# stijnherfst/Tyrant

Hardware: AMD Instinct MI355X
Metric: Mrays/s at 1080p 8spp (higher is better)
Workload: dtype f32

## Files before the change

tyrant_amd/csrc/hip/traverse.hpp:

```cpp
#pragma once

#include <type_traits>

#include <hip/hip_runtime.h>

#include "vecmath.hpp"

namespace tyr {

constexpr uint32_t kRefLeaf = 0x80000000u;
constexpr uint32_t kRefDone = 0xFFFFFFFFu;
constexpr uint32_t kRefPop = 0xFFFFFFFEu;
constexpr int kStackSize = 64;
constexpr uint32_t kMaxLeafPrims = 31;
constexpr uint32_t kMaxPrimOffset = 1u << 26;
constexpr uint32_t kStagedNodes = 64;
constexpr uint32_t kQuadOrderShift = 25;
constexpr uint32_t kQuadIndexMask = (1u << kQuadOrderShift) - 1u;

struct DevScene {
	const float4* quads;
	uint32_t quadRootRef;
	uint32_t nQuads;
	uint32_t nStaged;
	uint32_t quadMaxStack;
	const float4* nodes;
	const float4* tris;
	float rootMin[3];
	float rootMax[3];
	uint32_t rootRef;
	uint32_t nPairs;
	uint32_t nPrims;
};

#ifdef __HIPCC__

struct RayConst {
	f3 o, d, inv;
	bool nx, ny, nz;
};

__device__ __forceinline__ RayConst make_ray(f3 o, f3 d) {
	RayConst r;
	r.o = o;
	r.d = d;
	r.inv = mk3(1.f / d.x, 1.f / d.y, 1.f / d.z);
	r.nx = r.inv.x < 0;
	r.ny = r.inv.y < 0;
	r.nz = r.inv.z < 0;
	return r;
}

__device__ __forceinline__ bool slab_test(const RayConst& r, float lox, float hix, float loy, float hiy, float loz, float hiz, float lowest, float& tMinOut) {
	float tMin = (lox - r.o.x) * r.inv.x;
	float tMax = (hix - r.o.x) * r.inv.x;
	const float tyMin = (loy - r.o.y) * r.inv.y;
	const float tyMax = (hiy - r.o.y) * r.inv.y;
	bool ok = !(tMin > tyMax || tyMin > tMax);
	if (tyMin > tMin)
		tMin = tyMin;
	if (tyMax < tMax)
		tMax = tyMax;
	const float tzMin = (loz - r.o.z) * r.inv.z;
	const float tzMax = (hiz - r.o.z) * r.inv.z;
	ok = ok && !(tMin > tzMax || tzMin > tMax);
	if (tzMin > tMin)
		tMin = tzMin;
	if (tzMax < tMax)
		tMax = tzMax;
	tMinOut = tMin;
	return ok && (tMin < lowest) && (tMax > 0);
}

struct TriData {
	float4 a, b, c;
};
__device__ __forceinline__ TriData triangle_load(const float4* __restrict__ tris, uint32_t prim) {
	TriData d;
	d.a = tris[3 * prim + 0];
	d.b = tris[3 * prim + 1];
	d.c = tris[3 * prim + 2];
	return d;
}
__device__ __forceinline__ float triangle_test(const TriData& d, const RayConst& r);
__device__ __forceinline__ float triangle_test(const float4* __restrict__ tris, uint32_t prim, const RayConst& r) { return triangle_test(triangle_load(tris, prim), r); }
__device__ __forceinline__ float triangle_test(const TriData& d, const RayConst& r) {
	const float4 a = d.a, b = d.b, c = d.c;
	const f3 vert = mk3(a.x, a.y, a.z);
	const f3 e1 = mk3(a.w, b.x, b.y);
	const f3 e2 = mk3(b.z, b.w, c.x);
	const f3 pvec = cross(r.d, e2);
	const float det = dot(e1, pvec);
	if (det < 0.0000001f)
		return 0.0f;
	const float invDet = 1 / det;
	const f3 tvec = r.o - vert;
	const float u = dot(tvec, pvec) * invDet;
	if (u < 0 || u > 1)
		return 0.0f;
	const f3 qvec = cross(tvec, e1);
	const float v = dot(r.d, qvec) * invDet;
	if (v < 0 || u + v > 1)
		return 0.0f;
	return dot(e2, qvec) * invDet;
}
__device__ __forceinline__ float triangle_test_uv(const TriData& d, const RayConst& r, float& uOut, float& vOut) {
	const float4 a = d.a, b = d.b, c = d.c;
	const f3 vert = mk3(a.x, a.y, a.z);
	const f3 e1 = mk3(a.w, b.x, b.y);
	const f3 e2 = mk3(b.z, b.w, c.x);
	const f3 pvec = cross(r.d, e2);
	const float det = dot(e1, pvec);
	if (det < 0.0000001f)
		return 0.0f;
	const float invDet = 1 / det;
	const f3 tvec = r.o - vert;
	const float u = dot(tvec, pvec) * invDet;
	if (u < 0 || u > 1)
		return 0.0f;
	const f3 qvec = cross(tvec, e1);
	const float v = dot(r.d, qvec) * invDet;
	if (v < 0 || u + v > 1)
		return 0.0f;
	uOut = u;
	vOut = v;
	return dot(e2, qvec) * invDet;
}

__device__ __forceinline__ float triangle_test_select(const TriData& d, const RayConst& r) {
	const float4 a = d.a, b = d.b, c = d.c;
	const f3 vert = mk3(a.x, a.y, a.z);
	const f3 e1 = mk3(a.w, b.x, b.y);
	const f3 e2 = mk3(b.z, b.w, c.x);
	const f3 pvec = cross(r.d, e2);
	const float det = dot(e1, pvec);
	const bool out0 = det < 0.0000001f;
	const float invDet = 1 / det;
	const f3 tvec = r.o - vert;
	const float u = dot(tvec, pvec) * invDet;
	const bool out1 = u < 0 || u > 1;
	const f3 qvec = cross(tvec, e1);
	const float v = dot(r.d, qvec) * invDet;
	const bool out2 = v < 0 || u + v > 1;
	const float t = dot(e2, qvec) * invDet;
	return (out0 || out1 || out2) ? 0.0f : t;
}

template <int LDS_DEPTH>
struct TravStack {
	static constexpr int kBlockThreads = 256;
	static constexpr int kSpill = kStackSize - LDS_DEPTH;
	uint2* lds;
	uint32_t* spillRef;
	float* spillT;
	int n;
	uint32_t topRef;
	float topT;
	bool hasTop;
	bool overflow;
	__device__ __forceinline__ void bind(uint2* ldsColumn, uint32_t* refs, float* ts) {
		lds = ldsColumn;
		spillRef = refs;
		spillT = ts;
	}
	__device__ __forceinline__ void reset() {
		n = 0;
		hasTop = false;
		overflow = false;
	}
	__device__ __forceinline__ void push(uint32_t r, float t) {
		if (hasTop) {
			if (LDS_DEPTH > 0 && n < LDS_DEPTH) {
				lds[n * kBlockThreads] = make_uint2(topRef, __float_as_uint(topT));
				++n;
			} else if (n < kStackSize - 1) {
				spillRef[n - LDS_DEPTH] = topRef;
				spillT[n - LDS_DEPTH] = topT;
				++n;
			} else {
				overflow = true;
			}
		}
		topRef = r;
		topT = t;
		hasTop = true;
	}
	__device__ __forceinline__ bool pop(uint32_t& r, float& t) {
		if (hasTop) {
			r = topRef;
			t = topT;
			hasTop = false;
			return true;
		}
		if (n == 0)
			return false;
		--n;
		if (LDS_DEPTH > 0 && n < LDS_DEPTH) {
			const uint2 e = lds[n * kBlockThreads];
			r = e.x;
			t = __uint_as_float(e.y);
		} else {
			r = spillRef[n - LDS_DEPTH];
			t = spillT[n - LDS_DEPTH];
		}
		return true;
	}
};

template <int LDS_DEPTH, bool WITH_T = true>
struct LdsStack {
	static constexpr int kBlockThreads = 256;
	typedef typename std::conditional<WITH_T, uint2, uint32_t>::type entry_t;
#if defined(__HIP_DEVICE_COMPILE__)
	typedef __attribute__((address_space(3))) entry_t* lds_column_t;
#else
	typedef entry_t* lds_column_t;
#endif
	lds_column_t lds;
	uint32_t* spillRef;
	float* spillT;
	int n;
	bool overflow;
	__device__ __forceinline__ void bind(entry_t* ldsColumn, uint32_t* refs, float* ts) {
		lds = (lds_column_t)ldsColumn;
		spillRef = refs;
		spillT = ts;
	}
	__device__ __forceinline__ void reset() {
		n = 0;
		overflow = false;
	}
	__device__ __forceinline__ void lds_put(int d, uint32_t r, float t) {
		if constexpr (WITH_T)
			lds[d * kBlockThreads] = make_uint2(r, __float_as_uint(t));
		else
			lds[d * kBlockThreads] = r;
	}
	__device__ __forceinline__ void lds_get(int d, uint32_t& r, float& t) {
		if constexpr (WITH_T) {
			const uint2 e = lds[d * kBlockThreads];
			r = e.x;
			t = __uint_as_float(e.y);
		} else {
			r = lds[d * kBlockThreads];
			t = -__builtin_inff();
		}
	}
	__device__ __forceinline__ void push(uint32_t r, float t) {
		if (LDS_DEPTH > 0 && n < LDS_DEPTH) {
			lds_put(n, r, t);
			++n;
		} else if (n < kStackSize) {
			spillRef[n - LDS_DEPTH] = r;
			if (WITH_T)
				spillT[n - LDS_DEPTH] = t;
			++n;
		} else {
			overflow = true;
		}
	}
	__device__ __forceinline__ bool pop(uint32_t& r, float& t) {
		if (n == 0)
			return false;
		if (LDS_DEPTH > 0 && __builtin_amdgcn_ballot_w64(n > LDS_DEPTH) == 0ull) {
			--n;
			lds_get(n, r, t);
			return true;
		}
		--n;
		if (LDS_DEPTH > 0 && n < LDS_DEPTH) {
			lds_get(n, r, t);
		} else {
			r = spillRef[n - LDS_DEPTH];
			t = WITH_T ? spillT[n - LDS_DEPTH] : -__builtin_inff();
		}
		return true;
	}
	__device__ __forceinline__ void pop_select(bool popping, uint32_t& ref, float bound) {
		if (LDS_DEPTH > 0 && __builtin_amdgcn_ballot_w64(popping && n > LDS_DEPTH) == 0ull) {
			const bool take = popping && n > 0;
			uint32_t r;
			float t;
			lds_get(take ? n - 1 : 0, r, t);
			ref = popping ? (n == 0 ? kRefDone : (t < bound ? r : kRefPop)) : ref;
			n = take ? n - 1 : n;
			return;
		}
		if (popping) {
			if (n == 0) {
				ref = kRefDone;
			} else {
				--n;
				uint32_t r;
				float t;
				if (LDS_DEPTH > 0 && n < LDS_DEPTH) {
					lds_get(n, r, t);
				} else {
					r = spillRef[n - LDS_DEPTH];
					t = WITH_T ? spillT[n - LDS_DEPTH] : -__builtin_inff();
				}
				if (t < bound)
					ref = r;
			}
		}
	}
	__device__ __forceinline__ void push_ranked(const uint32_t* ref, const float* t, const unsigned long long* hit, const uint32_t* rank, uint32_t hr, uint32_t first) {
		if (LDS_DEPTH >= 3 && __builtin_amdgcn_ballot_w64(n > LDS_DEPTH - 3) == 0ull) {
			const uint32_t after = hr >> 1;
#pragma unroll
			for (int s = 0; s < 4; ++s)
				if (__builtin_amdgcn_inverse_ballot_w64(hit[s]) && rank[s] != first)
					lds_put(n + (int)__popc(after >> rank[s]), ref[s], t[s]);
			n += (int)__popc(hr) - (hr != 0u ? 1 : 0);
			return;
		}
		uint32_t oref[4];
		float ot[4];
#pragma unroll
		for (uint32_t k = 1; k < 4; ++k) {
			oref[k] = rank[0] == k ? ref[0] : rank[1] == k ? ref[1] : rank[2] == k ? ref[2] : ref[3];
			ot[k] = rank[0] == k ? t[0] : rank[1] == k ? t[1] : rank[2] == k ? t[2] : t[3];
		}
		if ((hr & 8u) && (hr & 7u))
			push(oref[3], ot[3]);
		if ((hr & 4u) && (hr & 3u))
			push(oref[2], ot[2]);
		if ((hr & 2u) && (hr & 1u))
			push(oref[1], ot[1]);
	}
	__device__ __forceinline__ void push3(unsigned long long ma, uint32_t ra, float ta, unsigned long long mb, uint32_t rb, float tb, unsigned long long mc, uint32_t rc, float tc) {
		if (LDS_DEPTH >= 3 && __builtin_amdgcn_ballot_w64(n > LDS_DEPTH - 3) == 0ull) {
			if (__builtin_amdgcn_inverse_ballot_w64(ma)) {
				lds_put(n, ra, ta);
				++n;
			}
			if (__builtin_amdgcn_inverse_ballot_w64(mb)) {
				lds_put(n, rb, tb);
				++n;
			}
			if (__builtin_amdgcn_inverse_ballot_w64(mc)) {
				lds_put(n, rc, tc);
				++n;
			}
			return;
		}
		if (__builtin_amdgcn_inverse_ballot_w64(ma))
			push(ra, ta);
		if (__builtin_amdgcn_inverse_ballot_w64(mb))
			push(rb, tb);
		if (__builtin_amdgcn_inverse_ballot_w64(mc))
			push(rc, tc);
	}
};

struct PairTest {
	uint32_t nearRef, farRef;
	float nearT, farT;
	bool nearHit, farHit;
	bool synthetic;
};

__device__ __forceinline__ PairTest test_pair(const float4* __restrict__ nodes, uint32_t idx, const RayConst& r, float dist) {
	const float4 qx = nodes[4 * idx + 0];
	const float4 qy = nodes[4 * idx + 1];
	const float4 qz = nodes[4 * idx + 2];
	const float4 qr = nodes[4 * idx + 3];
	const uint32_t leftRef = __float_as_uint(qr.x), rightRef = __float_as_uint(qr.y), axis = __float_as_uint(qr.z);
	float tL, tR;
	const bool hL = slab_test(r, r.nx ? qx.y : qx.x, r.nx ? qx.x : qx.y, r.ny ? qy.y : qy.x, r.ny ? qy.x : qy.y, r.nz ? qz.y : qz.x, r.nz ? qz.x : qz.y, dist, tL);
	const bool hR = slab_test(r, r.nx ? qx.w : qx.z, r.nx ? qx.z : qx.w, r.ny ? qy.w : qy.z, r.ny ? qy.z : qy.w, r.nz ? qz.w : qz.z, r.nz ? qz.z : qz.w, dist, tR);
	const bool rightFirst = (axis == 0) ? r.nx : (axis == 1) ? r.ny : (axis == 2) ? r.nz : false;
	PairTest p;
	p.nearRef = rightFirst ? rightRef : leftRef;
	p.farRef = rightFirst ? leftRef : rightRef;
	p.nearT = rightFirst ? tR : tL;
	p.farT = rightFirst ? tL : tR;
	p.nearHit = rightFirst ? hR : hL;
	p.farHit = rightFirst ? hL : hR;
	p.synthetic = (axis == 3);
	if (p.synthetic) {
		p.nearHit = true;
		p.farHit = true;
		p.farT = -__builtin_inff();
	}
	return p;
}


typedef float v2f __attribute__((ext_vector_type(2)));
__device__ __forceinline__ bool slab_fast(const RayConst& r, float lox, float hix, float loy, float hiy, float loz, float hiz, float lowest, float& tMinOut) {
	const float ox = r.o.x, oy = r.o.y, oz = r.o.z, ix = r.inv.x, iy = r.inv.y, iz = r.inv.z;
	v2f x = { lox, hix }, y = { loy, hiy }, z = { loz, hiz };
	x = (x - ox) * ix;
	y = (y - oy) * iy;
	z = (z - oz) * iz;
	const float tMin = __builtin_fmaxf(__builtin_fmaxf(__builtin_fminf(x.x, x.y), __builtin_fminf(y.x, y.y)), __builtin_fminf(z.x, z.y));
	const float tMax = __builtin_fminf(__builtin_fminf(__builtin_fmaxf(x.x, x.y), __builtin_fmaxf(y.x, y.y)), __builtin_fmaxf(z.x, z.y));
	tMinOut = tMin;
	return (tMin <= tMax) && (tMin < lowest) && (tMax > 0);
}
typedef unsigned long long lanemask;
__device__ __forceinline__ lanemask slab_fast_mask(const RayConst& r, float lox, float hix, float loy, float hiy, float loz, float hiz, float lowest, float& tMinOut) {
	const float ox = r.o.x, oy = r.o.y, oz = r.o.z, ix = r.inv.x, iy = r.inv.y, iz = r.inv.z;
	v2f x = { lox, hix }, y = { loy, hiy }, z = { loz, hiz };
	x = (x - ox) * ix;
	y = (y - oy) * iy;
	z = (z - oz) * iz;
	const float tMin = __builtin_fmaxf(__builtin_fmaxf(__builtin_fminf(x.x, x.y), __builtin_fminf(y.x, y.y)), __builtin_fminf(z.x, z.y));
	const float tMax = __builtin_fminf(__builtin_fminf(__builtin_fmaxf(x.x, x.y), __builtin_fmaxf(y.x, y.y)), __builtin_fmaxf(z.x, z.y));
	tMinOut = tMin;
	return __builtin_amdgcn_ballot_w64(tMin <= tMax) & __builtin_amdgcn_ballot_w64(tMin < lowest) & __builtin_amdgcn_ballot_w64(tMax > 0);
}
__device__ __forceinline__ bool ray_is_regular(const RayConst& r) {
	return (fabsf(r.inv.x) < __builtin_inff()) && (fabsf(r.inv.y) < __builtin_inff()) && (fabsf(r.inv.z) < __builtin_inff());
}
__device__ __forceinline__ PairTest test_pair_fast(const float4* __restrict__ nodes, uint32_t idx, const RayConst& r, float dist) {
	const float4 qx = nodes[4 * idx + 0];
	const float4 qy = nodes[4 * idx + 1];
	const float4 qz = nodes[4 * idx + 2];
	const float4 qr = nodes[4 * idx + 3];
	const uint32_t leftRef = __float_as_uint(qr.x), rightRef = __float_as_uint(qr.y), axis = __float_as_uint(qr.z);
	float tL, tR;
	const bool hL = slab_fast(r, qx.x, qx.y, qy.x, qy.y, qz.x, qz.y, dist, tL);
	const bool hR = slab_fast(r, qx.z, qx.w, qy.z, qy.w, qz.z, qz.w, dist, tR);
	const bool rightFirst = (axis == 0) ? r.nx : (axis == 1) ? r.ny : (axis == 2) ? r.nz : false;
	PairTest p;
	p.nearRef = rightFirst ? rightRef : leftRef;
	p.farRef = rightFirst ? leftRef : rightRef;
	p.nearT = rightFirst ? tR : tL;
	p.farT = rightFirst ? tL : tR;
	p.nearHit = rightFirst ? hR : hL;
	p.farHit = rightFirst ? hL : hR;
	p.synthetic = (axis == 3);
	if (p.synthetic) {
		p.nearHit = true;
		p.farHit = true;
		p.farT = -__builtin_inff();
	}
	return p;
}


__device__ __forceinline__ lanemask lanes_where(bool p) { return __builtin_amdgcn_ballot_w64(p); }
__device__ __forceinline__ bool lane_in(lanemask m) { return __builtin_amdgcn_inverse_ballot_w64(m); }
__device__ __forceinline__ lanemask mask_select(lanemask sel, lanemask a, lanemask b) { return (sel & a) | (~sel & b); }

__device__ __forceinline__ bool ref_is_leaf(uint32_t ref) { return (ref & kRefLeaf) && ref < kRefPop; }
__device__ __forceinline__ lanemask lanes_traversing(uint32_t ref) { return __builtin_amdgcn_ballot_w64((int)ref >= 0) | __builtin_amdgcn_ballot_w64(ref == kRefPop); }
__device__ __forceinline__ lanemask lanes_at_leaf(uint32_t ref) { return __builtin_amdgcn_ballot_w64((ref & kRefLeaf) != 0u) & __builtin_amdgcn_ballot_w64(ref < kRefPop); }

struct QuadHits {
	uint32_t ref[4];
	float t[4];
	lanemask hit[4];
};

template <bool FAST>
__device__ __forceinline__ lanemask slab_any(const RayConst& r, float lox, float hix, float loy, float hiy, float loz, float hiz, float lowest, float& tOut) {
	if (FAST)
		return slab_fast_mask(r, lox, hix, loy, hiy, loz, hiz, lowest, tOut);
	return lanes_where(slab_test(r, r.nx ? hix : lox, r.nx ? lox : hix, r.ny ? hiy : loy, r.ny ? loy : hiy, r.nz ? hiz : loz, r.nz ? loz : hiz, lowest, tOut));
}

template <bool FAST, bool ORDERED, bool STAGED = false, int STAGE_STRIDE = (int)kStagedNodes>
__device__ __forceinline__ QuadHits test_quad(const float4* __restrict__ quads, uint32_t ref, const RayConst& r, float dist, const float4* staged = nullptr, uint32_t nStaged = 0) {
	const uint32_t idx = ref & kQuadIndexMask;
	const float4* q = quads + 8 * idx;
	const uint32_t meta = ref >> kQuadOrderShift;
	float4 x01, x23, y01, y23, z01, z23, rf;
	if (STAGED && idx < nStaged) {
#if defined(__HIP_DEVICE_COMPILE__)
		typedef __attribute__((address_space(3))) const float4* lds_f4;
		const lds_f4 c = (lds_f4)staged + idx;
#else
		const float4* c = staged + idx;
#endif
		x01 = c[0 * STAGE_STRIDE], x23 = c[1 * STAGE_STRIDE], y01 = c[2 * STAGE_STRIDE], y23 = c[3 * STAGE_STRIDE];
		z01 = c[4 * STAGE_STRIDE], z23 = c[5 * STAGE_STRIDE], rf = c[6 * STAGE_STRIDE];
		__asm__ volatile("" : "+v"(rf.x));
	} else {
		x01 = q[0], x23 = q[1], y01 = q[2], y23 = q[3], z01 = q[4], z23 = q[5], rf = q[6];
	}
	const uint32_t r0 = __float_as_uint(rf.x), r1 = __float_as_uint(rf.y), r2 = __float_as_uint(rf.z), r3 = __float_as_uint(rf.w);
	float t0, t1, t2, t3;
	const lanemask H0 = slab_any<FAST>(r, x01.x, x01.y, y01.x, y01.y, z01.x, z01.y, dist, t0);
	const lanemask H1 = slab_any<FAST>(r, x01.z, x01.w, y01.z, y01.w, z01.z, z01.w, dist, t1);
	const lanemask H2 = slab_any<FAST>(r, x23.x, x23.y, y23.x, y23.y, z23.x, z23.y, dist, t2);
	const lanemask H3 = slab_any<FAST>(r, x23.z, x23.w, y23.z, y23.w, z23.z, z23.w, dist, t3);
	if (!ORDERED) {
		QuadHits o;
		o.ref[0] = r0, o.ref[1] = r1, o.ref[2] = r2, o.ref[3] = r3;
		o.t[0] = t0, o.t[1] = t1, o.t[2] = t2, o.t[3] = t3;
		o.hit[0] = H0, o.hit[1] = H1, o.hit[2] = H2, o.hit[3] = H3;
		return o;
	}
	const uint32_t signBits = (r.nx ? 1u : 0u) | (r.ny ? 2u : 0u) | (r.nz ? 4u : 0u);
	const uint32_t aT = meta & 3u, aL = (meta >> 2) & 3u, aR = (meta >> 4) & 3u;
	const bool bT = ((signBits >> aT) & 1u) != 0u;
	const bool bL = ((signBits >> aL) & 1u) != 0u;
	const bool bR = ((signBits >> aR) & 1u) != 0u;
	const lanemask BT = lanes_where(bT), BL = lanes_where(bL), BR = lanes_where(bR);
	const uint32_t lr0 = bL ? r1 : r0, lr1 = bL ? r0 : r1;
	const float lt0 = bL ? t1 : t0, lt1 = bL ? t0 : t1;
	const lanemask LH0 = mask_select(BL, H1, H0), LH1 = mask_select(BL, H0, H1);
	const uint32_t rr0 = bR ? r3 : r2, rr1 = bR ? r2 : r3;
	const float rt0 = bR ? t3 : t2, rt1 = bR ? t2 : t3;
	const lanemask RH0 = mask_select(BR, H3, H2), RH1 = mask_select(BR, H2, H3);
	QuadHits o;
	o.ref[0] = bT ? rr0 : lr0;
	o.ref[1] = bT ? rr1 : lr1;
	o.ref[2] = bT ? lr0 : rr0;
	o.ref[3] = bT ? lr1 : rr1;
	o.t[0] = bT ? rt0 : lt0;
	o.t[1] = bT ? rt1 : lt1;
	o.t[2] = bT ? lt0 : rt0;
	o.t[3] = bT ? lt1 : rt1;
	o.hit[0] = mask_select(BT, RH0, LH0);
	o.hit[1] = mask_select(BT, RH1, LH1);
	o.hit[2] = mask_select(BT, LH0, RH0);
	o.hit[3] = mask_select(BT, LH1, RH1);
	return o;
}

__device__ __forceinline__ void quad_ranks(uint32_t ref, uint32_t signBits, uint32_t* rank) {
	const uint32_t bT = __builtin_amdgcn_ubfe(signBits, __builtin_amdgcn_ubfe(ref, kQuadOrderShift, 2u), 1u);
	const uint32_t bL = __builtin_amdgcn_ubfe(signBits, __builtin_amdgcn_ubfe(ref, kQuadOrderShift + 2u, 2u), 1u);
	const uint32_t bR = __builtin_amdgcn_ubfe(signBits, __builtin_amdgcn_ubfe(ref, kQuadOrderShift + 4u, 2u), 1u);
	const uint32_t xL = (bT << 1) | bL, xR = (bT << 1) | bR;
	rank[0] = xL;
	rank[1] = xL ^ 1u;
	rank[2] = xR ^ 2u;
	rank[3] = xR ^ 3u;
}

struct VisitCount {
	uint32_t nodes, tris;
};

template <bool COUNT, class Stack>
__device__ __forceinline__ bool bvh_closest(const DevScene& sc, const RayConst& r, float& dist, int& prim, Stack& st, VisitCount& vc) {
	bool hit = false;
	st.reset();
	uint32_t ref;
	{
		float t0;
		const bool ok = slab_test(r, r.nx ? sc.rootMax[0] : sc.rootMin[0], r.nx ? sc.rootMin[0] : sc.rootMax[0], r.ny ? sc.rootMax[1] : sc.rootMin[1], r.ny ? sc.rootMin[1] : sc.rootMax[1],
			r.nz ? sc.rootMax[2] : sc.rootMin[2], r.nz ? sc.rootMin[2] : sc.rootMax[2], dist, t0);
		if (COUNT)
			vc.nodes += 1;
		ref = ok ? sc.rootRef : kRefDone;
	}
	while (ref != kRefDone) {
		while ((int)ref >= 0) {
			const PairTest p = test_pair(sc.nodes, ref, r, dist);
			if (COUNT && !p.synthetic)
				vc.nodes += 2;
			if (p.nearHit) {
				if (p.farHit)
					st.push(p.farRef, p.farT);
				ref = p.nearRef;
			} else if (p.farHit) {
				ref = p.farRef;
			} else {
				ref = kRefDone;
				uint32_t pr;
				float pt;
				while (st.pop(pr, pt)) {
					if (pt < dist) {
						ref = pr;
						break;
					}
				}
			}
		}
		if (ref == kRefDone)
			break;
		const uint32_t off = ref & (kMaxPrimOffset - 1);
		const uint32_t cnt = ((ref >> 26) & 31u) + 1u;
		for (uint32_t i = 0; i < cnt; ++i) {
			const float t = triangle_test(sc.tris, off + i, r);
			if (COUNT)
				vc.tris += 1;
			if (t > kEpsilon && t < dist && ((dist - t) > kEpsilon)) {
				prim = (int)(off + i);
				dist = t;
				hit = true;
			}
		}
		ref = kRefDone;
		uint32_t pr;
		float pt;
		while (st.pop(pr, pt)) {
			if (pt < dist) {
				ref = pr;
				break;
			}
		}
	}
	return hit;
}

template <bool COUNT, class Stack>
__device__ __forceinline__ bool bvh_any(const DevScene& sc, const RayConst& r, float closest, Stack& st, VisitCount& vc) {
	st.reset();
	uint32_t ref;
	{
		float t0;
		const bool ok = slab_test(r, r.nx ? sc.rootMax[0] : sc.rootMin[0], r.nx ? sc.rootMin[0] : sc.rootMax[0], r.ny ? sc.rootMax[1] : sc.rootMin[1], r.ny ? sc.rootMin[1] : sc.rootMax[1],
			r.nz ? sc.rootMax[2] : sc.rootMin[2], r.nz ? sc.rootMin[2] : sc.rootMax[2], closest, t0);
		if (COUNT)
			vc.nodes += 1;
		ref = ok ? sc.rootRef : kRefDone;
	}
	const float kFailed = __builtin_inff();
	while (ref != kRefDone) {
		while ((int)ref >= 0) {
			const PairTest p = test_pair(sc.nodes, ref, r, closest);
			if (COUNT && !p.synthetic) {
				vc.nodes += 1;
				st.push(p.farRef, p.farHit ? p.farT : kFailed);
				ref = p.nearHit ? p.nearRef : kRefDone;
			} else {
				if (p.nearHit) {
					if (p.farHit)
						st.push(p.farRef, p.farT);
					ref = p.nearRef;
				} else if (p.farHit) {
					ref = p.farRef;
				} else {
					ref = kRefDone;
				}
			}
			if (ref == kRefDone) {
				uint32_t pr;
				float pt;
				while (st.pop(pr, pt)) {
					if (COUNT)
						vc.nodes += 1;
					if (pt < closest) {
						ref = pr;
						break;
					}
				}
			}
		}
		if (ref == kRefDone)
			break;
		const uint32_t off = ref & (kMaxPrimOffset - 1);
		const uint32_t cnt = ((ref >> 26) & 31u) + 1u;
		for (uint32_t i = 0; i < cnt; ++i) {
			const float t = triangle_test(sc.tris, off + i, r);
			if (COUNT)
				vc.tris += 1;
			if (t > kEpsilon && ((closest - t) > kEpsilon))
				return true;
		}
		ref = kRefDone;
		uint32_t pr;
		float pt;
		while (st.pop(pr, pt)) {
			if (COUNT)
				vc.nodes += 1;
			if (pt < closest) {
				ref = pr;
				break;
			}
		}
	}
	return false;
}

#endif

}
```

tyrant_amd/csrc/hip/traverse_flat.hip:

```cpp
#include "device_common.hpp"
#include "scan_wave.hpp"

namespace tyr {

constexpr uint32_t kTraceBlockWide = 768;
#define TYR_FLAT_WAVES_PER_EU (STACK_LDS <= 8 ? 6 : STACK_LDS <= 12 ? 5 : STACK_LDS <= 16 ? 3 : 2)


#ifdef TYR_QUAD_STATS
constexpr bool kLoopStats = true;
#else
constexpr bool kLoopStats = false;
#endif
#if defined(TYR_QUAD_STATS) || defined(TYR_LAUNCH_ANATOMY)
constexpr bool kAnatomy = true;
#else
constexpr bool kAnatomy = false;
#endif
#define TYR_DBG(i)                                                     \
	if (COUNT || kLoopStats) {                                         \
		const unsigned long long m_ = __ballot(1);                     \
		if (lane == (uint32_t)__ffsll((long long)m_) - 1) {            \
			dbg[i] += 1;                                               \
			dbg[i + 1] += __popcll(m_);                                \
// ... 412 lines not shown
constexpr int kWideStackEntries = 4 * 12;

#ifdef TYR_LAUNCH_ANATOMY
#define TYR_WIDE_STEPS_PARAM , uint32_t& wideSteps
#define TYR_WIDE_STEPS_ARG , wideSteps
#else
#define TYR_WIDE_STEPS_PARAM
#define TYR_WIDE_STEPS_ARG
#endif
constexpr uint32_t kWideRegular = 1u, kWideHitTri = 2u, kWideShadow = 4u, kWideOccluded = 8u, kWideLive = 16u;
template <int STACK_LDS>
__device__ __attribute__((noinline, cold)) uint32_t wide_drain(unsigned long long kernarg, typename LdsStack<STACK_LDS, true>::lds_column_t smem_, float rox, float roy, float roz, float rdx, float rdy, float rdz, float rix, float riy, float riz, float dist,
                                                         uint32_t ref, uint32_t slot, int prim, uint32_t flags, int n, uint32_t passes TYR_WIDE_STEPS_PARAM) {
	const unsigned long long ka = (unsigned long long)(uint32_t)__builtin_amdgcn_readfirstlane((int)(uint32_t)kernarg) | ((unsigned long long)(uint32_t)__builtin_amdgcn_readfirstlane((int)(uint32_t)(kernarg >> 32)) << 32);
	const FrameParams& P = *(const FrameParams*)(const __attribute__((address_space(4))) FrameParams*)ka;
	const uint32_t lane = lane_id();
	const unsigned long long below = (1ull << lane) - 1ull;
	const bool live = (flags & kWideLive) != 0u;
	uint32_t visible = 0;
	const uint32_t sub = lane & 3u, grp = lane >> 2;
	const unsigned long long lm = __ballot(live);
	const uint32_t nl = (uint32_t)__popcll(lm);
	const uint32_t told = (uint32_t)__builtin_amdgcn_ds_permute(live ? (int)(__popcll(lm & below) << 2) : 63 * 4, (int)lane);
	bool gActive = grp < nl;
	const uint32_t asked = (uint32_t)__builtin_amdgcn_ds_bpermute((int)(grp << 2), (int)told);
	const uint32_t srcLane = gActive ? asked : lane;
	const int pull = (int)(srcLane << 2);
	auto pull_f = [&](float v) { return __uint_as_float((uint32_t)__builtin_amdgcn_ds_bpermute(pull, (int)__float_as_uint(v))); };
	auto pull_u = [&](uint32_t v) { return (uint32_t)__builtin_amdgcn_ds_bpermute(pull, (int)v); };
	rox = pull_f(rox), roy = pull_f(roy), roz = pull_f(roz);
	rdx = pull_f(rdx), rdy = pull_f(rdy), rdz = pull_f(rdz);
	rix = pull_f(rix), riy = pull_f(riy), riz = pull_f(riz);
	dist = pull_f(dist);
	ref = pull_u(ref);
	slot = pull_u(slot);
	prim = (int)pull_u((uint32_t)prim);
	const uint32_t fl = pull_u(flags);
	const bool regular = (fl & kWideRegular) != 0u, isShadow = (fl & kWideShadow) != 0u;
	bool hitTri = (fl & kWideHitTri) != 0u, occluded = (fl & kWideOccluded) != 0u;
	n = (int)pull_u((uint32_t)n);
	typedef typename LdsStack<STACK_LDS, true>::entry_t entry_t;
	typedef typename LdsStack<STACK_LDS, true>::lds_column_t lds_ptr_t;
	const lds_ptr_t column0 = smem_ + (threadIdx.x >> 8) * (STACK_LDS * kBlock) + (threadIdx.x & 255u & ~63u);
	entry_t moved[STACK_LDS / 4];
#pragma unroll
	for (int row = 0; row < STACK_LDS / 4; ++row) {
		const int e = 4 * row + (int)sub;
		moved[row] = (gActive && e < n) ? column0[e * kBlock + srcLane] : entry_t{};
	}
	wave_lds_order();
#pragma unroll
	for (int row = 0; row < STACK_LDS / 4; ++row)
		if (gActive && 4 * row + (int)sub < n)
			column0[row * kBlock + lane] = moved[row];
	wave_lds_order();
	const lds_ptr_t gstack = column0 + (lane & ~3u);
	auto entry_at = [&](int e) { return gstack + (((uint32_t)e >> 2) * kBlock + ((uint32_t)e & 3u)); };
	const RayConst r = { mk3(rox, roy, roz), mk3(rdx, rdy, rdz), mk3(rix, riy, riz), rix < 0, riy < 0, riz < 0 };
	const uint32_t signBits = (r.nx ? 1u : 0u) | (r.ny ? 2u : 0u) | (r.nz ? 4u : 0u);
	const uint32_t boxAt = (sub >> 1) * 16u + (sub & 1u) * 8u, refAt = 96u + 4u * sub, groupBits = kQuadOrderShift + 2u + 2u * (sub >> 1);
	const float4* const quads = P.scene.quads;
	const float4* const tris = P.scene.tris;
	const lanemask shadowM = __ballot(isShadow);
	lanemask act = __ballot(gActive), hitM = __ballot(hitTri), occM = __ballot(occluded);
	bool wideOverflow = false;
	const bool allRegular = (act & ~__ballot(regular)) == 0ull;
	while (act != 0ull) {
		if (kGuardPasses && ++passes > kMaxPasses)
			break;
#ifdef TYR_LAUNCH_ANATOMY
		wideSteps += 1;
#endif
		{
			const bool popping = lane_in(act & lanes_where(ref == kRefPop));
			const bool has = n > 0;
			const entry_t e = *entry_at(has ? n - 1 : 0);
			const uint32_t popped = !has ? kRefDone : (__uint_as_float(e.y) < dist ? e.x : kRefPop);
			ref = popping ? popped : ref;
			n = (popping && has) ? n - 1 : n;
		}
		const lanemask nodeM = act & lanes_where((int)ref >= 0);
		if (nodeM != 0ull) {
			const bool atNode = lane_in(nodeM);
			const uint32_t node = (atNode ? (ref & kQuadIndexMask) : 0u) * 128u;
			const float2 bx = gload_f2(quads, node + boxAt);
			const float2 by = gload_f2(quads, node + boxAt + 32u);
			const float2 bz = gload_f2(quads, node + boxAt + 64u);
			const uint32_t cref = gload_u(quads, node + refAt);
			float t;
			lanemask H;
			if (allRegular)
				H = slab_fast_mask(r, bx.x, bx.y, by.x, by.y, bz.x, bz.y, dist, t);
			else
				H = lanes_where(slab_test(r, r.nx ? bx.y : bx.x, r.nx ? bx.x : bx.y, r.ny ? by.y : by.x, r.ny ? by.x : by.y, r.nz ? bz.y : bz.x, r.nz ? bz.x : bz.y, dist, t));
			const bool h = lane_in(H & nodeM);
			const uint32_t bT = __builtin_amdgcn_ubfe(signBits, __builtin_amdgcn_ubfe(ref, kQuadOrderShift, 2u), 1u);
			const uint32_t bG = __builtin_amdgcn_ubfe(signBits, __builtin_amdgcn_ubfe(ref, groupBits, 2u), 1u);
			const uint32_t rank = sub ^ ((bT << 1) | bG);
			const uint32_t hr = quad_or(h ? (1u << rank) : 0u);
			const bool nearest = h && (hr & (0u - hr)) == (1u << rank);
			const int e = n + (int)__popc(hr >> rank >> 1);
			if (h && !nearest && e < kWideStackEntries)
				*entry_at(e) = make_uint2(cref, __float_as_uint(t));
			const int n2 = n + (int)__popc(hr) - (hr != 0u ? 1 : 0);
			wideOverflow = wideOverflow || (nodeM & lanes_where(n2 > kWideStackEntries)) != 0ull;
			const uint32_t next = quad_or(nearest ? cref : 0u);
			ref = atNode ? (hr == 0u ? kRefPop : next) : ref;
			n = atNode ? (n2 > kWideStackEntries ? kWideStackEntries : n2) : n;
		}
		const lanemask leafM = act & lanes_at_leaf(ref);
		if (leafM != 0ull) {
			const bool atLeaf = lane_in(leafM);
			const uint32_t off = ref & (kMaxPrimOffset - 1);
			const uint32_t cnt = atLeaf ? ((ref >> 26) & 31u) + 1u : 0u;
			lanemask inM = 0ull;
			for (uint32_t base = 0; __ballot(base < cnt) != 0ull; base += 4u) {
				const uint32_t i = base + sub;
				const bool mine = i < cnt;
				const TriData td = triangle_gload(tris, mine ? off + i : 0u);
				float tm = triangle_test_select(td, r);
				tm = mine ? tm : 0.0f;
				const float tk[4] = { quad_bcast_f<0>(tm), quad_bcast_f<1>(tm), quad_bcast_f<2>(tm), quad_bcast_f<3>(tm) };
				uint32_t took = 4u;
#pragma unroll
				for (uint32_t k = 0; k < 4u; ++k) {
					const float t = tk[k];
					const lanemask in = lanes_where(t > kEpsilon) & lanes_where((dist - t) > kEpsilon);
					const lanemask closer = in & ~shadowM;
					inM |= in;
					hitM |= closer;
					dist = lane_in(closer) ? t : dist;
					took = lane_in(closer) ? k : took;
				}
				prim = took != 4u ? (int)(off + base + took) : prim;
			}
			const lanemask foundM = inM & shadowM & leafM;
			occM |= foundM;
			ref = atLeaf ? (lane_in(foundM) ? kRefDone : kRefPop) : ref;
		}
		const lanemask finM = act & lanes_where(ref == kRefDone);
		if (finM != 0ull) {
			if (lane_in(finM) && sub == 0u) {
				if (isShadow) {
					if (!lane_in(occM)) {
						const v4f_t c = ((const TYR_GLOBAL v4f_t*)P.shadowPrev.color)[slot];
						accumulate_pixel(P.blit, __float_as_int(((const TYR_GLOBAL v4f_t*)P.shadowPrev.dyz_cd_ix)[slot].w), mk3(c.x, c.y, c.z), 0);
						visible += 1;
					}
				} else if (lane_in(hitM)) {
					((TYR_GLOBAL v2f_t*)P.work.hit)[slot] = v2f_t{ dist, __uint_as_float((uint32_t)prim) };
				}
			}
			act &= ~finM;
		}
	}
	return visible | (wideOverflow ? 0x80000000u : 0u) | (kGuardPasses && passes > kMaxPasses ? 0x40000000u : 0u);
}

template <int STACK_LDS, uint32_t kTraceBlock>
#define TYR_TRACE_VIEW(name) const FrameParams& name = kernarg_view<FrameParams>();
__global__ void __launch_bounds__(kTraceBlock, (kTraceBlock == kTraceBlockWide ? 6 : TYR_FLAT_WAVES_PER_EU)) k_trace_flat(const FrameParams P) {
	constexpr bool COUNT = false;
	__shared__ typename LdsStack<STACK_LDS, true>::entry_t smem_[STACK_LDS * kTraceBlock];
	uint32_t spillRef_[kStackSize - STACK_LDS];
	float spillT_[kStackSize - STACK_LDS];
	LdsStack<STACK_LDS, true> st;
	st.bind(smem_ + (threadIdx.x >> 8) * (STACK_LDS * kBlock) + (threadIdx.x & 255u), spillRef_, spillT_);
	st.reset();
	__shared__ float4 stagedNodes[7 * kStagedNodes];
	__shared__ uint32_t blockNext;
	const uint32_t nStaged = P.scene.nStaged;
	for (uint32_t i = threadIdx.x; i < 7 * nStaged; i += kTraceBlock) {
		const uint32_t v = i / nStaged, n = i - v * nStaged;
		stagedNodes[v * kStagedNodes + n] = P.scene.quads[8 * n + v];
	}
	const uint32_t lane = lane_id();
	const unsigned long long below = (1ull << lane) - 1ull;
	[[maybe_unused]] uint32_t tripsFeed = 0;
	const uint32_t nExt = P.traceShadow == 2u ? 0u : queue_extent(P.segWork);
	const uint32_t nItems = nExt + (P.traceShadow != 0u ? queue_extent(P.kcPrev->seg) : 0u);
	const DevScene& sc = P.scene;
	float rox = 0.f, roy = 0.f, roz = 0.f, rdx = 0.f, rdy = 0.f, rdz = 0.f, rix = 0.f, riy = 0.f, riz = 0.f;
	bool regular = true, allRegular = true;
	float dist = 0.0f;
	uint32_t ref = kRefDone, slot = 0;
	int prim = 0;
	bool hitTri = false, live = false, overflow = false;
	bool isShadow = false, occluded = false;
	uint32_t visible = 0;
	uint32_t dbg[16] = {};
	uint32_t steps = 0;
	[[maybe_unused]] unsigned long long tExhausted = 0ull, tWide = 0ull;
	[[maybe_unused]] uint32_t liveAtExhaustion = 0, liveAtWide = 0, tripsAfter = 0, passesAfter = 0, wideSteps = 0;
	const unsigned long long tStart = kAnatomy ? __builtin_amdgcn_s_memrealtime() : 0ull;
	constexpr uint32_t kNoPending = 0xffffffffu;
	uint32_t pendIdx = kNoPending;
	auto flush_visible = [&]() {
		TYR_TRACE_VIEW(P)
		float4 c = make_float4(0.f, 0.f, 0.f, 0.f);
		int px = 0;
		if (pendIdx != kNoPending) {
			c = P.shadowPrev.color[pendIdx];
			px = __float_as_int(P.shadowPrev.dyz_cd_ix[pendIdx].w);
		}
		accumulate_pixels_wave(P.blit, px, mk3(c.x, c.y, c.z), 0);
		pendIdx = kNoPending;
	};
	const uint32_t perBlock = static_range(nItems, P.staticShare);
	const uint32_t dynBase = perBlock * gridDim.x;
	const uint32_t blockBegin = blockIdx.x * perBlock, blockEnd = blockBegin + perBlock;
	ChunkFeed feed;
	feed.init(nItems - dynBase, P.ticketChunk);
	bool staticDone = (perBlock == 0);
	if (threadIdx.x == 0)
		blockNext = blockBegin;
	__syncthreads();
	if (P.scanPrevInTrace == 1u) {
		const uint32_t wavesPerBlock = kTraceBlock / 64u;
		scan_blocks_by_wave(P.survFlag, const_cast<unsigned long long*>(P.vPrev.word), const_cast<uint32_t*>(P.vPrev.pre), const_cast<uint32_t*>(P.vPrev.blk), &P.k->scan_blocks_done,
		                    *P.scanLivePrev, (threadIdx.x >> 6) * gridDim.x + blockIdx.x, gridDim.x * wavesPerBlock, P.retireGhosts != 0u);
	}
	bool exhausted = nItems == 0;
	bool wide = false;
	const uint32_t wideLimit = (P.wideDrain != 0u && P.scene.quadMaxStack <= (uint32_t)kWideStackEntries) ? kWideRays : 0u;
	uint32_t passes = 0;

	for (;;) {
		if (kGuardPasses && ++passes > kMaxPasses)
			break;
		const unsigned long long idleMask = __ballot(!live);
		const uint32_t nIdle = __popcll(idleMask);
		if (!exhausted && nIdle >= P.refillMinIdle) {
			TYR_TRACE_VIEW(P)
			const DevScene& sc = P.scene;
			const uint32_t rank = __popcll(idleMask & below);
			uint32_t s = 0;
			bool fed = false;
			uint32_t got = 0;
			if (!staticDone) {
				uint32_t base = 0;
				if (lane == 0)
					base = atomicAdd(&blockNext, nIdle);
				base = (uint32_t)__builtin_amdgcn_readfirstlane((int)__shfl(base, 0, 64));
				const uint32_t avail = base < blockEnd ? blockEnd - base : 0u;
				got = avail < nIdle ? avail : nIdle;
				if (!live && rank < got) {
					s = static_slot(base + rank, blockBegin, P.staticInterleave != 0u);
					fed = true;
				}
				staticDone = (base + nIdle >= blockEnd);
			}
			while (staticDone && got < nIdle) {
				if (!feed.refill(P.k->extend_chunks, nItems - dynBase, lane)) {
					exhausted = true;
					if (kAnatomy && tExhausted == 0ull) {
						tExhausted = __builtin_amdgcn_s_memrealtime();
						liveAtExhaustion = (uint32_t)__popcll(__ballot(live)) + got;
					}
					break;
				}
				const uint32_t avail = feed.end - feed.next, room = nIdle - got;
				const uint32_t take = avail < room ? avail : room;
				if (!live && rank >= got && rank < got + take) {
					s = dynBase + feed.next + (rank - got);
					fed = true;
				}
				feed.next += take;
				got += take;
			}
			if (__ballot(pendIdx != kNoPending) != 0ull)
				flush_visible();
			if (fed) {
				TYR_DBG(6)
				float4 a;
				float by, bz, bound;
				bool blocked = false;
				if (s < nExt) {
					a = P.work.o_dx[s];
					const float2 b = P.work.dyz[s];
					const float2 h = P.work.hit[s];
					by = b.x, bz = b.y, bound = h.x;
					slot = s;
					isShadow = false;
				} else {
					const uint32_t idx = s - nExt;
					a = P.shadowPrev.o_dx[idx];
					const float4 b = P.shadowPrev.dyz_cd_ix[idx];
					blocked = reinterpret_cast<const float*>(&P.shadowPrev.color[idx])[3] != 0.0f;
					by = b.x, bz = b.y, bound = b.z;
					slot = idx;
					isShadow = true;
				}
				const RayConst nr = make_ray(mk3(a.x, a.y, a.z), mk3(a.w, by, bz));
				rox = nr.o.x, roy = nr.o.y, roz = nr.o.z, rdx = nr.d.x, rdy = nr.d.y, rdz = nr.d.z, rix = nr.inv.x, riy = nr.inv.y, riz = nr.inv.z;
				regular = ray_is_regular(nr);
				dist = bound;
				hitTri = false;
				occluded = blocked;
				st.reset();
				ref = blocked ? kRefDone : root_ref(sc, nr, dist);
				if (ref != kRefDone)
					ref = sc.quadRootRef;
				live = (ref != kRefDone) || (isShadow && !blocked);
			}
			if (!exhausted && (uint32_t)__popcll(__ballot(live && ref != kRefDone)) < P.minTraversing)
				if (__ballot(live && ref == kRefDone) == 0ull)
					continue;
		}
		{
			const uint32_t nLiveNow = (uint32_t)__popcll(__ballot(live));
			if (exhausted && nLiveNow <= wideLimit && __ballot(live && st.n > STACK_LDS) == 0ull) {
				wide = nLiveNow != 0u;
				if (kAnatomy) {
					tWide = __builtin_amdgcn_s_memrealtime();
					liveAtWide = nLiveNow;
				}
				break;
			}
			if (kAnatomy && exhausted)
				passesAfter += 1;
			if (nLiveNow == 0u)
				continue;
		}
		allRegular = (__ballot(live && !regular) == 0ull);
		const RayConst r = { mk3(rox, roy, roz), mk3(rdx, rdy, rdz), mk3(rix, riy, riz), rix < 0, riy < 0, riz < 0 };
		const uint32_t signBits = (r.nx ? 1u : 0u) | (r.ny ? 2u : 0u) | (r.nz ? 4u : 0u);
		for (;;) {
			const uint32_t nTrav = __popcll(lanes_traversing(ref));
			if (nTrav == 0)
				break;
			if (nTrav < P.minTraversing) {
				const bool anyLeaf = lanes_at_leaf(ref) != 0ull;
				const bool canRefill = !exhausted && (uint32_t)__popcll(__ballot(!live || ref == kRefDone)) >= P.refillMinIdle;
				if (anyLeaf || canRefill)
					break;
			}
			if (kAnatomy && exhausted)
				tripsAfter += 1;
			if (kAnatomy && !exhausted)
				tripsFeed += 1;
			if (kLoopStats && ref == kRefPop) {
				TYR_DBG(2)
			}
			st.pop_select(ref == kRefPop, ref, dist);
			if ((int)ref >= 0) {
				TYR_DBG(0)
				if (kLoopStats)
					steps += 1;
				const QuadHits q = allRegular ? test_quad<true, false, true>(sc.quads, ref, r, dist, stagedNodes, nStaged) : test_quad<false, false, true>(sc.quads, ref, r, dist, stagedNodes, nStaged);
				uint32_t rank[4];
				quad_ranks(ref, signBits, rank);
				const uint32_t hr = (lane_in(q.hit[0]) ? 1u << rank[0] : 0u) | (lane_in(q.hit[1]) ? 1u << rank[1] : 0u) | (lane_in(q.hit[2]) ? 1u << rank[2] : 0u) | (lane_in(q.hit[3]) ? 1u << rank[3] : 0u);
				const uint32_t first = (uint32_t)__ffs((int)hr) - 1u;
				st.push_ranked(q.ref, q.t, q.hit, rank, hr, first);
				ref = rank[0] == first ? q.ref[0] : rank[1] == first ? q.ref[1] : rank[2] == first ? q.ref[2] : rank[3] == first ? q.ref[3] : kRefPop;
			}
		}
		{
			const bool atLeaf = ref_is_leaf(ref);
			const unsigned long long B0 = __ballot(atLeaf);
			if (B0 != 0ull) {
				const uint32_t off = ref & (kMaxPrimOffset - 1);
				const uint32_t cnt = atLeaf ? ((ref >> 26) & 31u) + 1u : 0u;
				const unsigned long long B1 = __ballot(cnt > 1u), B2 = __ballot(cnt > 2u), B3 = __ballot(cnt > 3u);
				const uint32_t n0 = (uint32_t)__popcll(B0), n1 = (uint32_t)__popcll(B1), n2 = (uint32_t)__popcll(B2), n3 = (uint32_t)__popcll(B3);
				if (__ballot(cnt > 4u) == 0ull && n0 + n1 + n2 + n3 <= 63u) {
					const uint32_t base1 = n0, base2 = n0 + n1, base3 = n0 + n1 + n2;
					const uint32_t s0 = (uint32_t)__popcll(B0 & below), s1 = base1 + (uint32_t)__popcll(B1 & below), s2 = base2 + (uint32_t)__popcll(B2 & below), s3 = base3 + (uint32_t)__popcll(B3 & below);
					const uint32_t me = lane + 1u;
					uint32_t told = (uint32_t)__builtin_amdgcn_ds_permute((int)((cnt > 0u ? s0 : 63u) << 2), (int)(cnt > 0u ? me : 0u));
					if (n1)
						told |= (uint32_t)__builtin_amdgcn_ds_permute((int)((cnt > 1u ? s1 : 63u) << 2), (int)(cnt > 1u ? (me | (1u << 8)) : 0u));
					if (n2)
						told |= (uint32_t)__builtin_amdgcn_ds_permute((int)((cnt > 2u ? s2 : 63u) << 2), (int)(cnt > 2u ? (me | (2u << 8)) : 0u));
					if (n3)
						told |= (uint32_t)__builtin_amdgcn_ds_permute((int)((cnt > 3u ? s3 : 63u) << 2), (int)(cnt > 3u ? (me | (3u << 8)) : 0u));
					const bool item = lane < n0 + n1 + n2 + n3;
					const int from = (int)((item ? (told & 0xffu) - 1u : lane) << 2);
					auto pull = [&](float v) { return __uint_as_float((uint32_t)__builtin_amdgcn_ds_bpermute(from, (int)__float_as_uint(v))); };
					const uint32_t offO = (uint32_t)__builtin_amdgcn_ds_bpermute(from, (int)off);
					RayConst ro;
					ro.o = mk3(pull(rox), pull(roy), pull(roz));
					ro.d = mk3(pull(rdx), pull(rdy), pull(rdz));
					if ((COUNT || kLoopStats) && item) {
						TYR_DBG(4)
					}
					float tm = triangle_test_select(triangle_load(sc.tris, item ? offO + (told >> 8) : 0u), ro);
					tm = item ? tm : 0.0f;
					const float t0 = __uint_as_float((uint32_t)__builtin_amdgcn_ds_bpermute((int)(s0 << 2), (int)__float_as_uint(tm)));
					const float t1 = n1 ? __uint_as_float((uint32_t)__builtin_amdgcn_ds_bpermute((int)(s1 << 2), (int)__float_as_uint(tm))) : 0.0f;
					const float t2 = n2 ? __uint_as_float((uint32_t)__builtin_amdgcn_ds_bpermute((int)(s2 << 2), (int)__float_as_uint(tm))) : 0.0f;
					const float t3 = n3 ? __uint_as_float((uint32_t)__builtin_amdgcn_ds_bpermute((int)(s3 << 2), (int)__float_as_uint(tm))) : 0.0f;
					const float tk[4] = { t0, t1, t2, t3 };
					bool found = false;
#pragma unroll
					for (uint32_t i = 0; i < 4u; ++i) {
						const float t = tk[i];
						const bool in = i < cnt && !found && t > kEpsilon && ((dist - t) > kEpsilon);
						const bool closer = in && !isShadow && t < dist;
						found = found || (in && isShadow);
						prim = closer ? (int)(off + i) : prim;
						hitTri = hitTri || closer;
						dist = closer ? t : dist;
					}
					if (atLeaf) {
						occluded = occluded || found;
						ref = found ? kRefDone : kRefPop;
					}
				}
			}
		}
		if (ref_is_leaf(ref)) {
			const uint32_t off = ref & (kMaxPrimOffset - 1);
			const uint32_t cnt = ((ref >> 26) & 31u) + 1u;
			bool found = false;
			TriData tri = triangle_load(sc.tris, off);
			for (uint32_t i = 0; i < cnt && !found; ++i) {
				TYR_DBG(4)
				const TriData cur = tri;
				if (i + 1 < cnt)
					tri = triangle_load(sc.tris, off + i + 1);
				const float t = triangle_test(cur, r);
				if (isShadow) {
					found = (t > kEpsilon && ((dist - t) > kEpsilon));
				} else if (t > kEpsilon && t < dist && ((dist - t) > kEpsilon)) {
					prim = (int)(off + i);
					dist = t;
					hitTri = true;
				}
			}
			occluded = occluded || found;
			ref = found ? kRefDone : kRefPop;
		}
		if (live && ref == kRefDone) {
			if (isShadow) {
				if (!occluded) {
					pendIdx = slot;
					visible += 1;
				}
			} else {
				finish_extend_ray(P.work.hit, slot, hitTri, dist, prim);
			}
			overflow = overflow || st.overflow;
			live = false;
			if (kLoopStats) {
				atomicMax(&P.k->debug[12], (unsigned long long)steps);
				if (steps > 64)
					atomicAdd(&P.k->debug[9], 1ull);
				if (steps > 128)
					atomicAdd(&P.k->debug[10], 1ull);
				if (steps > 256)
					atomicAdd(&P.k->debug[11], 1ull);
				steps = 0;
			}
		}
	}
	flush_visible();
	TYR_TRACE_VIEW(PE)
	if (wide) {
		const uint32_t flags = (regular ? kWideRegular : 0u) | (hitTri ? kWideHitTri : 0u) | (isShadow ? kWideShadow : 0u) | (occluded ? kWideOccluded : 0u) | (live ? kWideLive : 0u);
		const uint32_t res = wide_drain<STACK_LDS>((unsigned long long)__builtin_amdgcn_kernarg_segment_ptr(), (typename LdsStack<STACK_LDS, true>::lds_column_t)smem_, rox, roy, roz, rdx, rdy, rdz, rix, riy, riz, dist, ref, slot, prim, flags, st.n, passes TYR_WIDE_STEPS_ARG);
		visible += res & 0x3fffffffu;
		overflow = overflow || (res & 0x80000000u) != 0u;
		if (res & 0x40000000u)
			passes = kMaxPasses + 1;
	}
	if (overflow)
		atomicOr(&PE.k->device_error, kErrStackOverflow);
	if (kGuardPasses && passes > kMaxPasses)
		atomicOr(&PE.k->device_error, kErrNoProgress);
	wave_add_u64(&PE.k->n_shadow_visible, visible);
	if (kLoopStats) {
		for (int i = 0; i < 9; ++i)
			wave_add_u64(&PE.k->debug[i], dbg[i]);
	}
	if (kAnatomy && lane == 0) {
		const unsigned long long tEnd = __builtin_amdgcn_s_memrealtime();
		atomicMax(&P.k->debug[13], ~tStart);
		atomicMax(&P.k->debug[14], ~(tExhausted ? tExhausted : tEnd));
		atomicMax(&P.k->debug[15], tEnd);
		const uint32_t w = blockIdx.x * (kTraceBlock / 64) + (threadIdx.x >> 6);
		if (w < P.N)
			P.next.hit[w] = make_float2((float)((tExhausted ? tExhausted : tEnd) - tStart) * 0.01f, (float)(tEnd - tStart) * 0.01f + (float)liveAtExhaustion * 0.0f);
		if (w < 8192u && 32768u < P.N) {
			P.next.hit[8192u + w] = make_float2(tWide ? (float)(tWide - tStart) * 0.01f : 0.0f, (float)(liveAtExhaustion + 256u * liveAtWide));
			P.next.hit[16384u + w] = make_float2((float)tripsAfter, (float)wideSteps);
			P.next.hit[24576u + w] = make_float2((float)passesAfter, (float)tripsFeed);
		}
	}
}

#undef TYR_DBG
#undef TYR_TRACE_VIEW


#define TYR_TRACE_STACK 12
void launch_trace(const FrameParams& P, uint32_t maxLive, uint32_t nSurvivors, uint32_t maxShadowPrev, const Tuning& t, int numCUs, LaunchCache& lc, hipStream_t stream) {
	launch_trace_prepasses(P, nSurvivors, maxShadowPrev, stream, maxLive);
	launch_trace_kernel(P, maxLive + maxShadowPrev, t, numCUs, lc, stream);
}
void launch_trace_kernel(const FrameParams& P, uint32_t items, const Tuning& t, int numCUs, LaunchCache& lc, hipStream_t stream) {
	if (t.wideBlockMinItems >= 0 && items >= (uint32_t)t.wideBlockMinItems)
		launch_in_stage((k_trace_flat<TYR_TRACE_STACK, kTraceBlockWide>), dim3(persistent_blocks(k_trace_flat<TYR_TRACE_STACK, kTraceBlockWide>, items, t, numCUs, lc.perCU[kLcTrace][1], kTraceBlockWide)), dim3(kTraceBlockWide), stream, P);
	else
		launch_in_stage((k_trace_flat<TYR_TRACE_STACK, (uint32_t)kBlock>), dim3(persistent_blocks(k_trace_flat<TYR_TRACE_STACK, (uint32_t)kBlock>, items, t, numCUs, lc.perCU[kLcTrace][0])), dim3(kBlock), stream, P);
}
void launch_trace_prepasses(const FrameParams& P, uint32_t nSurvivors, uint32_t maxShadowPrev, hipStream_t stream, uint32_t maxLive) {
	FrameParams Pc = P;
	Pc.kc = P.kcPrev;
	Pc.shadow = P.shadowPrev;
	if (P.prevFolded) {
		if (!P.prologueDone)
			launch_pad_holes(Pc, P.traceShadow != 2u, maxShadowPrev != 0, stream, P.traceShadow == 2u);
		return;
	}
	if (P.traceShadow != 2u)
		launch_extend_spheres(P, nSurvivors, stream, maxLive);
	if (maxShadowPrev != 0)
		launch_connect_spheres(Pc, maxShadowPrev, stream);
	if (P.traceShadow != 2u && nSurvivors == 0)
		launch_pad_holes(Pc, true, false, stream);
}

void launch_extend(const FrameParams& P0, uint32_t maxLive, uint32_t nSurvivors, bool countVisits, const Tuning& t, int numCUs, LaunchCache& lc, hipStream_t stream) {
	if (maxLive == 0)
		return;
	FrameParams P = P0;
	if (countVisits) {
		launch_extend_spheres(P, nSurvivors, stream, maxLive);
		P.raysPerBlock = kCountRaysPerBlock;
		const uint32_t blocks = (P.segCap * kSegs + kCountRaysPerBlock - 1) / kCountRaysPerBlock;
		launch_in_stage((k_extend_count<12>), dim3(blocks), dim3(kBlock), stream, P);
		return;
	}
	P.traceShadow = 0u;
	launch_trace(P, maxLive, nSurvivors, 0u, t, numCUs, lc, stream);
}
void launch_connect(const FrameParams& P0, uint32_t maxShadow, bool countVisits, const Tuning& t, int numCUs, LaunchCache& lc, hipStream_t stream) {
	if (maxShadow == 0)
		return;
	FrameParams P = P0;
	if (countVisits) {
		launch_connect_spheres(P, maxShadow, stream);
		P.raysPerBlock = kCountRaysPerBlock;
		const uint32_t blocks = (P.segCap * kSegs + kCountRaysPerBlock - 1) / kCountRaysPerBlock;
		launch_in_stage((k_connect_count<12>), dim3(blocks), dim3(kBlock), stream, P);
		return;
	}
	P.kcPrev = P.kc;
	P.shadowPrev = P.shadow;
	P.traceShadow = 2u;
	launch_trace(P, 0u, 0u, maxShadow, t, numCUs, lc, stream);
}

}
```

Before: 8594.

## Restructure stack pop/push spill paths and add scheduling barriers in quad test

Rewrites pop_select so lanes that must pop from the spill area do it in a side branch, after which all lanes take the branch-free LDS pop path. The slow push path now writes directly with rank-based offsets into LDS or spill memory instead of three sequential conditional pushes, and reports stack overflow through a callback that sets a device error flag. Adds empty asm barriers in test_quad and the refill loop to constrain instruction scheduling and keep LDS and global loads apart, and computes the idle-lane mask from two lane masks instead of a combined ballot. The aim is less divergence and less redundant control flow in the traversal inner loop, at the cost of an extra overflow check and possibly worse scheduling from the barriers.

```diff
diff --git a/tyrant_amd/csrc/hip/traverse.hpp b/tyrant_amd/csrc/hip/traverse.hpp
--- a/tyrant_amd/csrc/hip/traverse.hpp
+++ b/tyrant_amd/csrc/hip/traverse.hpp
@@ -277,34 +277,29 @@
 		return true;
 	}
 	__device__ __forceinline__ void pop_select(bool popping, uint32_t& ref, float bound) {
-		if (LDS_DEPTH > 0 && __builtin_amdgcn_ballot_w64(popping && n > LDS_DEPTH) == 0ull) {
-			const bool take = popping && n > 0;
-			uint32_t r;
-			float t;
-			lds_get(take ? n - 1 : 0, r, t);
-			ref = popping ? (n == 0 ? kRefDone : (t < bound ? r : kRefPop)) : ref;
-			n = take ? n - 1 : n;
-			return;
-		}
-		if (popping) {
-			if (n == 0) {
-				ref = kRefDone;
-			} else {
+		if (LDS_DEPTH == 0 || (__builtin_amdgcn_ballot_w64(popping) & __builtin_amdgcn_ballot_w64(n > LDS_DEPTH)) != 0ull) {
+			if (popping && n > LDS_DEPTH) {
 				--n;
-				uint32_t r;
-				float t;
-				if (LDS_DEPTH > 0 && n < LDS_DEPTH) {
-					lds_get(n, r, t);
-				} else {
-					r = spillRef[n - LDS_DEPTH];
-					t = WITH_T ? spillT[n - LDS_DEPTH] : -__builtin_inff();
-				}
-				if (t < bound)
-					ref = r;
-			}
-		}
-	}
-	__device__ __forceinline__ void push_ranked(const uint32_t* ref, const float* t, const unsigned long long* hit, const uint32_t* rank, uint32_t hr, uint32_t first) {
+				uint32_t r = spillRef[n - LDS_DEPTH];
+				float t = WITH_T ? spillT[n - LDS_DEPTH] : -__builtin_inff();
+				__asm__ volatile("" : "+v"(r), "+v"(t));
+				ref = t < bound ? r : ref;
+				popping = false;
+			}
+			if (LDS_DEPTH == 0) {
+				ref = popping ? kRefDone : ref;
+				return;
+			}
+		}
+		const bool take = popping && n > 0;
+		uint32_t r;
+		float t;
+		lds_get(take ? n - 1 : 0, r, t);
+		ref = popping ? (n == 0 ? kRefDone : (t < bound ? r : kRefPop)) : ref;
+		n = take ? n - 1 : n;
+	}
+	template <class OnOverflow>
+	__device__ __forceinline__ void push_ranked(const uint32_t* ref, const float* t, const unsigned long long* hit, const uint32_t* rank, uint32_t hr, uint32_t first, OnOverflow onOverflow) {
 		if (LDS_DEPTH >= 3 && __builtin_amdgcn_ballot_w64(n > LDS_DEPTH - 3) == 0ull) {
 			const uint32_t after = hr >> 1;
 #pragma unroll
@@ -314,19 +309,23 @@
 			n += (int)__popc(hr) - (hr != 0u ? 1 : 0);
 			return;
 		}
-		uint32_t oref[4];
-		float ot[4];
+		const uint32_t after = hr >> 1;
 #pragma unroll
-		for (uint32_t k = 1; k < 4; ++k) {
-			oref[k] = rank[0] == k ? ref[0] : rank[1] == k ? ref[1] : rank[2] == k ? ref[2] : ref[3];
-			ot[k] = rank[0] == k ? t[0] : rank[1] == k ? t[1] : rank[2] == k ? t[2] : t[3];
-		}
-		if ((hr & 8u) && (hr & 7u))
-			push(oref[3], ot[3]);
-		if ((hr & 4u) && (hr & 3u))
-			push(oref[2], ot[2]);
-		if ((hr & 2u) && (hr & 1u))
-			push(oref[1], ot[1]);
+		for (int s = 0; s < 4; ++s)
+			if (__builtin_amdgcn_inverse_ballot_w64(hit[s]) && rank[s] != first) {
+				const int d = n + (int)__popc(after >> rank[s]);
+				if (LDS_DEPTH > 0 && d < LDS_DEPTH) {
+					lds_put(d, ref[s], t[s]);
+				} else if (d < kStackSize) {
+					spillRef[d - LDS_DEPTH] = ref[s];
+					if (WITH_T)
+						spillT[d - LDS_DEPTH] = t[s];
+				}
+			}
+		const int n2 = n + (int)__popc(hr) - (hr != 0u ? 1 : 0);
+		if (n2 > kStackSize)
+			onOverflow();
+		n = n2 > kStackSize ? kStackSize : n2;
 	}
 	__device__ __forceinline__ void push3(unsigned long long ma, uint32_t ra, float ta, unsigned long long mb, uint32_t rb, float tb, unsigned long long mc, uint32_t rc, float tc) {
 		if (LDS_DEPTH >= 3 && __builtin_amdgcn_ballot_w64(n > LDS_DEPTH - 3) == 0ull) {
@@ -468,7 +467,8 @@
 	const float4* q = quads + 8 * idx;
 	const uint32_t meta = ref >> kQuadOrderShift;
 	float4 x01, x23, y01, y23, z01, z23, rf;
-	if (STAGED && idx < nStaged) {
+	const bool inLds = STAGED && idx < nStaged;
+	if (inLds) {
 #if defined(__HIP_DEVICE_COMPILE__)
 		typedef __attribute__((address_space(3))) const float4* lds_f4;
 		const lds_f4 c = (lds_f4)staged + idx;
@@ -478,7 +478,10 @@
 		x01 = c[0 * STAGE_STRIDE], x23 = c[1 * STAGE_STRIDE], y01 = c[2 * STAGE_STRIDE], y23 = c[3 * STAGE_STRIDE];
 		z01 = c[4 * STAGE_STRIDE], z23 = c[5 * STAGE_STRIDE], rf = c[6 * STAGE_STRIDE];
 		__asm__ volatile("" : "+v"(rf.x));
-	} else {
+	}
+	if (STAGED)
+		__asm__ volatile("" ::: "memory");
+	if (!inLds) {
 		x01 = q[0], x23 = q[1], y01 = q[2], y23 = q[3], z01 = q[4], z23 = q[5], rf = q[6];
 	}
 	const uint32_t r0 = __float_as_uint(rf.x), r1 = __float_as_uint(rf.y), r2 = __float_as_uint(rf.z), r3 = __float_as_uint(rf.w);
@@ -487,6 +490,8 @@
 	const lanemask H1 = slab_any<FAST>(r, x01.z, x01.w, y01.z, y01.w, z01.z, z01.w, dist, t1);
 	const lanemask H2 = slab_any<FAST>(r, x23.x, x23.y, y23.x, y23.y, z23.x, z23.y, dist, t2);
 	const lanemask H3 = slab_any<FAST>(r, x23.z, x23.w, y23.z, y23.w, z23.z, z23.w, dist, t3);
+	if (STAGED)
+		__asm__ volatile("" ::"v"(rf.w));
 	if (!ORDERED) {
 		QuadHits o;
 		o.ref[0] = r0, o.ref[1] = r1, o.ref[2] = r2, o.ref[3] = r3;
diff --git a/tyrant_amd/csrc/hip/traverse_flat.hip b/tyrant_amd/csrc/hip/traverse_flat.hip
--- a/tyrant_amd/csrc/hip/traverse_flat.hip
+++ b/tyrant_amd/csrc/hip/traverse_flat.hip
@@ -738,6 +738,7 @@
 				if (ref != kRefDone)
 					ref = sc.quadRootRef;
 				live = (ref != kRefDone) || (isShadow && !blocked);
+				__asm__ volatile("" : "+v"(dist));
 			}
 			if (!exhausted && (uint32_t)__popcll(__ballot(live && ref != kRefDone)) < P.minTraversing)
 				if (__ballot(live && ref == kRefDone) == 0ull)
@@ -767,7 +768,7 @@
 				break;
 			if (nTrav < P.minTraversing) {
 				const bool anyLeaf = lanes_at_leaf(ref) != 0ull;
-				const bool canRefill = !exhausted && (uint32_t)__popcll(__ballot(!live || ref == kRefDone)) >= P.refillMinIdle;
+				const bool canRefill = !exhausted && (uint32_t)__popcll(lanes_where(!live) | lanes_where(ref == kRefDone)) >= P.refillMinIdle;
 				if (anyLeaf || canRefill)
 					break;
 			}
@@ -788,7 +789,7 @@
 				quad_ranks(ref, signBits, rank);
 				const uint32_t hr = (lane_in(q.hit[0]) ? 1u << rank[0] : 0u) | (lane_in(q.hit[1]) ? 1u << rank[1] : 0u) | (lane_in(q.hit[2]) ? 1u << rank[2] : 0u) | (lane_in(q.hit[3]) ? 1u << rank[3] : 0u);
 				const uint32_t first = (uint32_t)__ffs((int)hr) - 1u;
-				st.push_ranked(q.ref, q.t, q.hit, rank, hr, first);
+				st.push_ranked(q.ref, q.t, q.hit, rank, hr, first, [] { atomicOr(&kernarg_view<FrameParams>().k->device_error, kErrStackOverflow); });
 				ref = rank[0] == first ? q.ref[0] : rank[1] == first ? q.ref[1] : rank[2] == first ? q.ref[2] : rank[3] == first ? q.ref[3] : kRefPop;
 			}
 		}
```

New measurement: 8600, median of 3. Within noise of the previous version (+0.1%).
